# Berghojo/bmhrl

Measured on AMD Instinct MI355X. Metric: caption-train steps/sec, higher is better.
Workload: dtype bf16; 1 GPU; BMHRL warmstart step (BASELINE configs[1]): B=16/GPU Tv=256 Ta=800 L=30 V=10172 N=2 d_model=1024 H=4 dropout=0.1; global_batch=16, parallelism=dp1, launch=hip-graph

## Files before the change

### bmhrl_amd/_lib.py

```python
from __future__ import annotations

import ctypes as C
import os

_HERE = os.path.dirname(os.path.abspath(__file__))
LIB_PATH = os.environ.get("BMHRL_HIP_LIB") or os.path.join(_HERE, "csrc", "libbmhrl_hip.so")

i32, i64, u64, f32, f64 = C.c_int32, C.c_int64, C.c_uint64, C.c_float, C.c_double
ptr = C.c_void_p


class RnnLayer(C.Structure):
    _fields_ = [("w_ih", C.c_void_p), ("w_hh", C.c_void_p), ("b_ih", C.c_void_p), ("b_hh", C.c_void_p),
                ("in_seq", C.c_void_p), ("in_ld", C.c_int64), ("in_dim", C.c_int32), ("gates", C.c_int32),
                ("seq_out", C.c_void_p), ("h", C.c_void_p * 2), ("c", C.c_void_p * 2),
                ("arelu_alpha", C.c_void_p), ("arelu_beta", C.c_void_p), ("xproj", C.c_void_p)]


class FusionTailParams(C.Structure):
    _fields_ = [(n, C.c_void_p) for n in ("gamma_ca", "beta_ca", "gamma_cv", "beta_cv", "a_v",
                                          "dgamma_ca", "dbeta_ca", "dgamma_cv", "dbeta_cv", "da_v")]


class GemmDesc(C.Structure):
# ... 114 lines not shown
    "bmhrl_consensus": [ptr, i64, i32, i32, i32, i64, i32, ptr, i32, ptr, ptr, ptr],
    "bmhrl_word_cost": [ptr, i64, ptr, i64, i64, f32, i32, i32, i32, i32, ptr, ptr, ptr, ptr, ptr, ptr, ptr, ptr],
    "bmhrl_lsa_match": [ptr, i64, i64, i64, ptr, i32, i32, i32, ptr, ptr],
    "bmhrl_word_loss": [ptr, ptr, ptr, ptr, ptr, ptr, ptr, f32, i32, i32, i32, i32, ptr, ptr, ptr, ptr],
    "bmhrl_word_loss_bwd": [ptr, i64, ptr, ptr, ptr, ptr, ptr, ptr, ptr, i64, i32, i32, i32, ptr],
    "bmhrl_proposal_assign": [ptr, i32, ptr, i32, f32, i32, i32, ptr, ptr, ptr, ptr, ptr],
    "bmhrl_proposal_head": [ptr, ptr, f32, i32, i32, i32, ptr, i64, i64, ptr, ptr, ptr, ptr, f32, f32, ptr, ptr, ptr, ptr, ptr,
                            ptr],
    "bmhrl_proposal_select": [ptr, i32, i64, ptr, i32, f32, ptr, ptr, ptr, i64, ptr],
    "bmhrl_tiou_hits": [ptr, i32, ptr, i32, ptr, ptr, ptr, i32, ptr, i32, i32, ptr, i64, ptr, i64, ptr],
    "bmhrl_tiou_pairs": [ptr, i32, ptr, i32, ptr, ptr, ptr, i32, f64, ptr, i64, ptr, i64, ptr],
    "bmhrl_crop_segments": [ptr, ptr, ptr, i32, i32, i32, ptr, ptr, i32, f32, i32, ptr, ptr, ptr, ptr, ptr],
    "bmhrl_rollout_advantage": [ptr, i64, i32, i32, i32, i64, ptr, i64, i32, ptr, ptr, ptr, ptr, ptr, i64, ptr, ptr],
    "bmhrl_policy_loss_fwd": [ptr, i64, ptr, ptr, ptr, f32, ptr, ptr, ptr, i64, i32, ptr],
    "bmhrl_policy_loss_bwd": [ptr, i64, ptr, ptr, ptr, f32, ptr, ptr, ptr, ptr, i64, i64, i32, ptr],
    "bmhrl_ngram_stats": [ptr, i32, ptr, i32, ptr, i32, ptr, ptr],
}

QUERIES = {
    "bmhrl_hip_arch": (C.c_char_p, []),
    "bmhrl_hip_abi_version": (C.c_int, []),
    "bmhrl_deterministic_enabled": (C.c_int, []),
    "bmhrl_layernorm_bwd_workspace": (C.c_int64, [i64, i32]),
    "bmhrl_attention_shared128_bwd_workspace": (C.c_int64, [i32, i32, i32]),
    "bmhrl_attention_max_keys": (C.c_int, []),
    "bmhrl_attention_config": (C.c_int, [i32, i32]),
    "bmhrl_attention_plan": (C.c_int, [i32, i32, i32, i32, i32, i64]),
    "bmhrl_attention_bwd_scores256_ok": (C.c_int, [i32, i32, i32, i64]),
    "bmhrl_memory_attention_ok": (C.c_int, [i32, i32, i32]),
    "bmhrl_small_attention_ok": (C.c_int, [i32, i32, i32]),
    "bmhrl_gemm_splits": (C.c_int, [i32, i32, i32, i32]),
    "bmhrl_gemm_plan": (C.c_int, [C.POINTER(GemmDesc), C.POINTER(i32)]),
    "bmhrl_gemm_group_plan": (C.c_int, [C.POINTER(GemmDesc), i32]),
    "bmhrl_gemm_f32_fast_path": (C.c_int, [C.POINTER(GemmDesc)]),
}


def _is_pointer(t) -> bool:
    return t is ptr or isinstance(t, type(C.POINTER(i32)))


PTR_SLOTS = {name: tuple(i for i, t in enumerate(argtypes) if _is_pointer(t))
             for name, argtypes in [*PROTOTYPES.items(), *((name, q[1]) for name, q in QUERIES.items())]}

_lib = None


def load() -> C.CDLL:
    global _lib
    if _lib is not None:
        return _lib
    if not os.path.exists(LIB_PATH):
        raise RuntimeError(
            f"{LIB_PATH} is missing: build it with `python -m bmhrl_amd.build` (hipcc --offload-arch=gfx950). "
            "bmhrl_amd has no CPU fallback.")
    import torch
    hip_rt = os.path.join(os.path.dirname(torch.__file__), "lib", "libamdhip64.so")
    if os.path.exists(hip_rt):
        C.CDLL(hip_rt, mode=C.RTLD_GLOBAL)
    lib = C.CDLL(LIB_PATH)

    def bind(name, restype, argtypes):
        try:
            fn = getattr(lib, name)
        except AttributeError:
            raise RuntimeError(f"{LIB_PATH} does not export {name}: it was built from older sources than this package; "
# ... 21 lines not shown
```

### bmhrl_amd/csrc/gemm.hip

```cpp
#include <cstdlib>
#include <algorithm>
#include <type_traits>

#include "common.h"
#include "../../include/bmhrl_hip.h"

namespace {

struct GemmArgs {
  int M, N, K, batch2;
  const bf16_t* A; long lda, a_sb1, a_sb2;
  const bf16_t* B; long ldb, b_sb1, b_sb2;
  float* C; long ldc, c_sb1, c_sb2;
  bf16_t* Cb; long ldcb, cb_sb1, cb_sb2;
  int epilogue; float alpha; int relu; int accumulate;
  const float* bias;
  const float* residual; long ldr, r_sb1, r_sb2;
  const uint8_t* mask; long mask_sb1, mask_sm;
  const float* rowvec; const float* rowvec2; long rv_sb1, rv_sb2;
  const bf16_t* aux; long ldaux, aux_sb1, aux_sb2;
  float dropout_p; uint64_t seed; const uint64_t* seed_dev; long drop_sb1, drop_sb2, drop_sm;
  float* colsum; long cs_sb2, bias_sb2, cs_sb1, bias_sb1;
  int tiles_m, splits, k_per_split, vec_ok, dbg, fast_bf16, fast_pd, fast_f32, tiles_mn;
  int xcd_chunk, group_m;
// ... 606 lines not shown
  r /= p.tiles_mn;
  gemm_body<TM, TN, AT, BT>(p, bx, r % p.splits, r / p.splits);
}


template <int N> struct IC { static constexpr int value = N; };
template <int I, int N, class F>
__device__ __forceinline__ void gsfor(F&& f) {
  if constexpr (I < N) {
    f(IC<I>{});
    gsfor<I + 1, N>(f);
  }
}
template <int IMM>
__device__ __forceinline__ void gemm_glds16(const char* src, char* dst) {
  __builtin_amdgcn_global_load_lds((const __attribute__((address_space(1))) void*)src,
                                   (__attribute__((address_space(3))) void*)dst, 16, IMM, 0);
}

template <int OFF>
__device__ __forceinline__ bf16x8 gemm_lds128(unsigned addr) {
  bf16x8 r;
  asm volatile("ds_read_b128 %0, %1 offset:%2" : "=v"(r) : "v"(addr), "n"(OFF));
  return r;
}
template <int OFF>
__device__ __forceinline__ bf16x4 gemm_ldstr(unsigned addr) {
  bf16x4 r;
  asm volatile("ds_read_b64_tr_b16 %0, %1 offset:%2" : "=v"(r) : "v"(addr), "n"(OFF));
  return r;
}

template <int TM, int TN, bool AT, bool BT, int NS>
__global__ __launch_bounds__(256, 2) void gemm_glds_kernel(const GemmArgs p) {
  constexpr int BM = 64 * TM, BN = 64 * TN;
  constexpr int A_BYTES = BM * BK * 2, B_BYTES = BN * BK * 2, STAGE_BYTES = A_BYTES + B_BYTES;
  constexpr int EPI_ELEMS = BM * (BN + 4) * 2;
  constexpr int SMEM_ELEMS = (NS * STAGE_BYTES / 2) > EPI_ELEMS ? (NS * STAGE_BYTES / 2) : EPI_ELEMS;

  __shared__ __attribute__((aligned(16))) bf16_t smem[SMEM_ELEMS];
  char* const sbase = reinterpret_cast<char*>(smem);
  const unsigned lds0 = (unsigned)(uintptr_t)(__attribute__((address_space(3))) char*)sbase;

  const int tid = threadIdx.x, lane = tid & 63;
  const int wave = __builtin_amdgcn_readfirstlane(tid >> 6);
  const int wm = wave >> 1, wn = wave & 1;
  const int r32 = lane & 31, h = lane >> 5;
  const int g1 = (lane >> 4) & 1, q4 = (lane & 15) >> 2, p4 = lane & 3;
  const int bz = blockIdx.z, b1 = bz / p.batch2, b2 = bz % p.batch2;
  int tile_m, tile_n;
  tile_of_block(p, (int)blockIdx.x, tile_m, tile_n);
  const int m0 = tile_m * BM, n0 = tile_n * BN;
  const char* __restrict__ Ag = reinterpret_cast<const char*>(p.A + b1 * p.a_sb1 + b2 * p.a_sb2);
  const char* __restrict__ Bg = reinterpret_cast<const char*>(p.B + b1 * p.b_sb1 + b2 * p.b_sb2);
  const int M8 = (p.M + 7) & ~7, N8 = (p.N + 7) & ~7;
  const int k_begin = blockIdx.y * p.k_per_split;
  const int k_end = min(p.K, k_begin + p.k_per_split);
  const int nk = (k_end - k_begin) / BK;
  if (nk <= 0) return;
  BMHRL_GSTAMP(0)

  constexpr int PA = A_BYTES / 1024 / 4, PB = B_BYTES / 1024 / 4;
  unsigned a_off[PA], b_off[PB];
  auto piece_off = [&](const bool trans, const int R, const int i, const int r0, const int rmax, const int rmax8, const long ld) {
    if (!trans) {
      const int row = wave * (R / 4) + 8 * i + (lane >> 3), pc = lane & 7;
      const int sc = pc ^ ((row >> 1) & 7);
      return (unsigned)((long)min(r0 + row, rmax - 1) * ld * 2 + sc * 16);
    }
    const int cpr = R / 8, rpp = 64 / cpr;
    const int krow = wave * 16 + rpp * i + lane / cpr, pc = lane % cpr;
    const int sc = pc ^ (R == 128 ? ((krow & 3) << 2) : (((krow >> 1) & 1) << 2));
    return (unsigned)((long)krow * ld * 2 + (long)min(r0 + sc * 8, rmax8 - 8) * 2);
  };
#pragma unroll
  for (int i = 0; i < PA; ++i) a_off[i] = piece_off(AT, BM, i, m0, p.M, M8, p.lda);
#pragma unroll
  for (int i = 0; i < PB; ++i) b_off[i] = piece_off(BT, BN, i, n0, p.N, N8, p.ldb);
  const long a_step = AT ? (long)BK * p.lda * 2 : (long)BK * 2, b_step = BT ? (long)BK * p.ldb * 2 : (long)BK * 2;
  const char* const a_k0 = Ag + (AT ? (long)k_begin * p.lda * 2 : (long)k_begin * 2);
  const char* const b_k0 = Bg + (BT ? (long)k_begin * p.ldb * 2 : (long)k_begin * 2);
  char* const a_dst = sbase + wave * PA * 1024;
  char* const b_dst = sbase + A_BYTES + wave * PB * 1024;
  auto stage = [&](auto st_, const int t) {
    constexpr int ST = decltype(st_)::value;
    auto sgpr_ptr = [](const char* q) {
      const uint64_t u = reinterpret_cast<uint64_t>(q);
      const uint32_t lo = __builtin_amdgcn_readfirstlane((uint32_t)u), hi = __builtin_amdgcn_readfirstlane((uint32_t)(u >> 32));
      return reinterpret_cast<const char*>(((uint64_t)hi << 32) | lo);
    };
    const char* ab = sgpr_ptr(a_k0 + (long)t * a_step);
    const char* bb = sgpr_ptr(b_k0 + (long)t * b_step);
    gsfor<0, PA>([&](auto i) {
      constexpr int I = decltype(i)::value;
      unsigned o = a_off[I];
      asm volatile("" : "+v"(o));
      gemm_glds16<0>(ab + o, a_dst + ST * STAGE_BYTES + I * 1024);
    });
    gsfor<0, PB>([&](auto i) {
      constexpr int I = decltype(i)::value;
      unsigned o = b_off[I];
      asm volatile("" : "+v"(o));
      gemm_glds16<0>(bb + o, b_dst + ST * STAGE_BYTES + I * 1024);
    });
  };

  constexpr int NA = AT ? TM : 4, NB = BT ? TN : 4;
  unsigned a_addr0[NA], b_addr0[NB];
  if constexpr (!AT) {
#pragma unroll
    for (int ks = 0; ks < 4; ++ks) a_addr0[ks] = lds0 + (wm * 32 * TM + r32) * 128 + (((2 * ks + h) ^ ((r32 >> 1) & 7)) << 4);
  } else {
    constexpr int RB = BM * 2;
#pragma unroll
    for (int i = 0; i < TM; ++i) {
      const int c = wm * 4 * TM + 4 * i + 2 * g1 + (p4 >> 1);
      const int sw = BM == 128 ? (q4 << 2) : (((q4 >> 1) & 1) << 2);
      a_addr0[i] = lds0 + (8 * h + q4) * RB + ((c ^ sw) << 4) + ((p4 & 1) << 3);
    }
  }
  if constexpr (!BT) {
#pragma unroll
    for (int ks = 0; ks < 4; ++ks) b_addr0[ks] = lds0 + A_BYTES + (wn * 32 * TN + r32) * 128 + (((2 * ks + h) ^ ((r32 >> 1) & 7)) << 4);
  } else {
    constexpr int RB = BN * 2;
#pragma unroll
    for (int i = 0; i < TN; ++i) {
      const int c = wn * 4 * TN + 4 * i + 2 * g1 + (p4 >> 1);
      const int sw = BN == 128 ? (q4 << 2) : (((q4 >> 1) & 1) << 2);
      b_addr0[i] = lds0 + A_BYTES + (8 * h + q4) * RB + ((c ^ sw) << 4) + ((p4 & 1) << 3);
    }
  }

  f32x16 acc[TM][TN];
#pragma unroll
  for (int i = 0; i < TM; ++i)
#pragma unroll
    for (int j = 0; j < TN; ++j)
#pragma unroll
      for (int r = 0; r < 16; ++r) acc[i][j][r] = 0.f;

  constexpr int RA = AT ? 2 : 1, RBn = BT ? 2 : 1;
  constexpr int PER_KS = TM * RA + TN * RBn;
  auto compute = [&](auto st_) {
    constexpr int ST = decltype(st_)::value;
    bf16x8 af[4][TM], bfr[4][TN];
    unsigned a_addr[1][NA], b_addr[1][NB];
#pragma unroll
    for (int i = 0; i < NA; ++i) a_addr[0][i] = a_addr0[i] + ST * STAGE_BYTES;
#pragma unroll
    for (int i = 0; i < NB; ++i) b_addr[0][i] = b_addr0[i] + ST * STAGE_BYTES;
    auto read_ks = [&](auto ks_) {
      constexpr int KS = decltype(ks_)::value;
      gsfor<0, TM>([&](auto i_) {
        constexpr int I = decltype(i_)::value;
        if constexpr (!AT) {
          af[KS][I] = gemm_lds128<I * 32 * 128>(a_addr[0][KS]);
        } else {
          constexpr int RB = BM * 2;
          af[KS][I] = join8(gemm_ldstr<KS * 16 * RB>(a_addr[0][I]), gemm_ldstr<(KS * 16 + 4) * RB>(a_addr[0][I]));
        }
      });
      gsfor<0, TN>([&](auto i_) {
        constexpr int I = decltype(i_)::value;
        if constexpr (!BT) {
          bfr[KS][I] = gemm_lds128<I * 32 * 128>(b_addr[0][KS]);
        } else {
          constexpr int RB = BN * 2;
          bfr[KS][I] = join8(gemm_ldstr<KS * 16 * RB>(b_addr[0][I]), gemm_ldstr<(KS * 16 + 4) * RB>(b_addr[0][I]));
        }
      });
    };
    read_ks(IC<0>{});
    read_ks(IC<1>{});
    gsfor<0, 4>([&](auto ks_) {
      constexpr int KS = decltype(ks_)::value;
      constexpr int LEFT = KS < 3 ? PER_KS : 0;
      __builtin_amdgcn_sched_barrier(0);
      bf16x8& a0 = af[KS][0];
      bf16x8& b0 = bfr[KS][0];
      bf16x8& a1 = af[KS][TM - 1];
      bf16x8& b1r = bfr[KS][TN - 1];
      if constexpr (TM == 2 && TN == 2) asm volatile("s_waitcnt lgkmcnt(%4)" : "+v"(a0), "+v"(a1), "+v"(b0), "+v"(b1r) : "n"(LEFT));
      else asm volatile("s_waitcnt lgkmcnt(%2)" : "+v"(a0), "+v"(b0) : "n"(LEFT));
      __builtin_amdgcn_sched_barrier(0);
#pragma unroll
      for (int mi = 0; mi < TM; ++mi)
#pragma unroll
        for (int ni = 0; ni < TN; ++ni)
          acc[mi][ni] = __builtin_amdgcn_mfma_f32_32x32x16_bf16(af[KS][mi], bfr[KS][ni], acc[mi][ni], 0, 0, 0);
      if constexpr (KS + 2 < 4) read_ks(IC<KS + 2>{});
    });
  };

  constexpr int PT = PA + PB;
  auto step = [&](auto st_, const int t) {
    constexpr int ST = decltype(st_)::value;
    constexpr int NXT = (ST + NS - 1) % NS;
    const bool more = t + NS - 1 < nk;
    if (more) stage(IC<NXT>{}, t + NS - 1);
    compute(st_);
    if (t + 1 < nk) {
      if (more && NS > 2) asm volatile("s_waitcnt vmcnt(%0)" ::"n"((NS - 2) * PT) : "memory");
      else asm volatile("s_waitcnt vmcnt(0)" ::: "memory");
      __builtin_amdgcn_s_barrier();
      asm volatile("" ::: "memory");
    }
  };
  gsfor<0, NS - 1>([&](auto i_) {
    if (decltype(i_)::value < nk) stage(i_, decltype(i_)::value);
  });
  BMHRL_GSTAMP(1)
  if (NS > 2 && nk > 1) asm volatile("s_waitcnt vmcnt(%0)" ::"n"((NS - 2) * PT) : "memory");
  if (NS == 2 || nk < NS - 1) asm volatile("s_waitcnt vmcnt(0)" ::: "memory");
  __builtin_amdgcn_s_barrier();
  asm volatile("" ::: "memory");
  BMHRL_GSTAMP(2)
  for (int t0 = 0; t0 < nk; t0 += NS) {
    gsfor<0, NS>([&](auto i_) {
      if (t0 + decltype(i_)::value < nk) step(i_, t0 + decltype(i_)::value);
    });
  }
  asm volatile("s_waitcnt lgkmcnt(0)" ::: "memory");
  __builtin_amdgcn_s_barrier();
  asm volatile("" ::: "memory");
  BMHRL_GSTAMP(3)
  gemm_epilogue<TM, TN, SMEM_ELEMS>(p, acc, smem, b1, b2, m0, n0, (int)blockIdx.y);
  BMHRL_GSTAMP(4)
}

template <bool AT, bool BT>
__global__ __launch_bounds__(512, 2) void gemm_glds8_kernel(const GemmArgs p) {
  constexpr int TM = 2, TN = 2, NS = 3, NW = 8;
  constexpr int BM = 128, BN = 128;
  constexpr int A_BYTES = BM * BK * 2, B_BYTES = BN * BK * 2, STAGE_BYTES = A_BYTES + B_BYTES;
  constexpr int EPI_ELEMS = BM * (BN + 4) * 2;
  constexpr int SMEM_ELEMS = (NS * STAGE_BYTES / 2) > EPI_ELEMS ? (NS * STAGE_BYTES / 2) : EPI_ELEMS;
  static_assert(4 * 64 * 256 <= SMEM_ELEMS * 2, "the partial tile of wave group 1 fits the stages");

  __shared__ __attribute__((aligned(16))) bf16_t smem[SMEM_ELEMS];
  char* const sbase = reinterpret_cast<char*>(smem);
  const unsigned lds0 = (unsigned)(uintptr_t)(__attribute__((address_space(3))) char*)sbase;

  const int tid = threadIdx.x, lane = tid & 63;
  const int wave = __builtin_amdgcn_readfirstlane(tid >> 6);
  const int grp = wave >> 2, w4 = wave & 3;
  const int wm = w4 >> 1, wn = w4 & 1;
  const int r32 = lane & 31, h = lane >> 5;
  const int g1 = (lane >> 4) & 1, q4 = (lane & 15) >> 2, p4 = lane & 3;
  const int bz = blockIdx.z, b1 = bz / p.batch2, b2 = bz % p.batch2;
  const int tile_m = blockIdx.x % p.tiles_m, tile_n = blockIdx.x / p.tiles_m;
  const int m0 = tile_m * BM, n0 = tile_n * BN;
  const char* __restrict__ Ag = reinterpret_cast<const char*>(p.A + b1 * p.a_sb1 + b2 * p.a_sb2);
  const char* __restrict__ Bg = reinterpret_cast<const char*>(p.B + b1 * p.b_sb1 + b2 * p.b_sb2);
  const int M8 = (p.M + 7) & ~7, N8 = (p.N + 7) & ~7;
  const int nk = p.K / BK;
  BMHRL_GSTAMP(0)

  constexpr int PA = A_BYTES / 1024 / NW, PB = B_BYTES / 1024 / NW;
  unsigned a_off[PA], b_off[PB];
  auto piece_off = [&](const bool trans, const int R, const int i, const int r0, const int rmax, const int rmax8, const long ld) {
// ... 153 lines not shown
  if (grp == 1) {
#pragma unroll
    for (int mi = 0; mi < TM; ++mi)
#pragma unroll
      for (int ni = 0; ni < TN; ++ni)
#pragma unroll
        for (int g = 0; g < 4; ++g) {
          f32x4 v;
#pragma unroll
          for (int e = 0; e < 4; ++e) v[e] = acc[mi][ni][4 * g + e];
          xch[((mi * TN + ni) * 4 + g) * 64] = v;
        }
  }
  __syncthreads();
  if (grp == 1) return;
#pragma unroll
  for (int mi = 0; mi < TM; ++mi)
#pragma unroll
    for (int ni = 0; ni < TN; ++ni)
#pragma unroll
      for (int g = 0; g < 4; ++g) {
        const f32x4 v = xch[((mi * TN + ni) * 4 + g) * 64];
#pragma unroll
        for (int e = 0; e < 4; ++e) acc[mi][ni][4 * g + e] += v[e];
      }
  __syncthreads();
  gemm_epilogue<TM, TN, SMEM_ELEMS, false>(p, acc, smem, b1, b2, m0, n0, 0);
  BMHRL_GSTAMP(4)
}

bool uses_glds(const GemmArgs& a, int a_trans, int b_trans) {
  static const int no_glds = getenv("BMHRL_GEMM_NOGLDS") ? atoi(getenv("BMHRL_GEMM_NOGLDS")) : 0;
  const long a_span = (a_trans ? 64 : (long)a.M) * a.lda * 2, b_span = (b_trans ? 64 : (long)a.N) * a.ldb * 2;
  return !no_glds && a.K % BK == 0 && a_span < (1l << 31) && b_span < (1l << 31) && a.M >= 8 && a.N >= 8;
}

enum { LOOP_REG = 0, LOOP_GLDS = 1, LOOP_GLDS8 = 2 };
enum { TILE_64 = 0, TILE_128 = 1, TILE_128x64 = 2 };
enum { SPLIT_NONE = 0, SPLIT_ATOMIC = 1, SPLIT_ORDERED = 2 };
enum { EPIPATH_FAST_BF16 = 0, EPIPATH_FAST_PD = 1, EPIPATH_GENERIC = 2 };
struct GemmPlan { int loop, tile, stages, splits, split_form, epi_path, vec_ok, ordered_colsum, fast_f32; };

template <int TM, int TN>
hipError_t launch(const GemmArgs& a, const GemmPlan& pl, int a_trans, int b_trans, int batch, hipStream_t s) {
  GemmArgs p = a;
  constexpr int BM = 64 * TM, BN = 64 * TN;
  const int splits = pl.splits;
  p.tiles_m = (a.M + BM - 1) / BM;
  const int tiles_n = (a.N + BN - 1) / BN;
  p.tiles_mn = p.tiles_m * tiles_n;
  p.xcd_chunk = p.group_m = 0;
  {
    static const int xcd = getenv("BMHRL_GEMM_XCD") ? atoi(getenv("BMHRL_GEMM_XCD")) : 0;
    if (xcd && p.tiles_mn % 8 == 0 && p.tiles_mn >= 64 && tiles_n >= 2) {
      const int chunk = p.tiles_mn / 8;
      int g = 1;
      while ((g + 1) * (g + 1) <= chunk && g + 1 <= p.tiles_m) ++g;
      while (g > 1 && chunk % g != 0) --g;
      if (xcd >= 2) g = xcd <= p.tiles_m ? xcd : p.tiles_m;
      p.xcd_chunk = chunk;
      p.group_m = g;
    }
  }
  p.splits = splits;
  p.dbg = getenv("BMHRL_GEMM_DBG") ? atoi(getenv("BMHRL_GEMM_DBG")) : 0;
  const int ktiles = (a.K + BK - 1) / BK;
  p.k_per_split = ((ktiles + splits - 1) / splits) * BK;
  dim3 grid(p.tiles_m * tiles_n, splits, batch), block(256);
  if constexpr (TM == 2 && TN == 2) {
    if (pl.loop == LOOP_GLDS8) {
      dim3 block8(512);
      if (!a_trans && !b_trans) hipLaunchKernelGGL((gemm_glds8_kernel<false, false>), grid, block8, 0, s, p);
      else if (!a_trans && b_trans) hipLaunchKernelGGL((gemm_glds8_kernel<false, true>), grid, block8, 0, s, p);
      else if (a_trans && !b_trans) hipLaunchKernelGGL((gemm_glds8_kernel<true, false>), grid, block8, 0, s, p);
// ... 156 lines not shown
                                       : d->residual ? (d->dropout_p > 0.f || !d->Cb) : (d->dropout_p == 0.f && !d->Cb);
  a.fast_f32 = fast_f32_on && d->C && d->epilogue == BMHRL_EPI_LINEAR && !d->mask && !d->aux && !d->rowvec && !d->rowvec2 &&
               !d->relu && !d->colsum && f32_combo && a.vec_ok;
  const bool out_ok = d->Cb && !d->C && !d->residual && !d->colsum && !d->accumulate && !d->bias && al(d->Cb, 16) &&
                      d->ldcb % 8 == 0 && d->cb_sb1 % 8 == 0 && d->cb_sb2 % 8 == 0 && d->rowvec;
  a.fast_pd = (d->epilogue == BMHRL_EPI_PROB && out_ok && d->rowvec2 && (!d->mask || d->mask_sm == 0) && !d->aux) ||
              (d->epilogue == BMHRL_EPI_DSCORE && out_ok && d->aux && al(d->aux, 16) && d->ldaux % 8 == 0 &&
               d->aux_sb1 % 8 == 0 && d->aux_sb2 % 8 == 0 && (!d->mask || d->mask_sm == 0));
  const bool can_split = d->allow_split_k && d->C && !d->Cb && d->epilogue == BMHRL_EPI_LINEAR && !d->relu && !d->mask &&
                         d->dropout_p == 0.f && (!d->accumulate || d->split_ws) && !d->colsum;
  tp = tile_plan(d->M, d->N, d->K, batch, can_split);
  a.split_ws = (tp.splits > 1 && d->split_ws && d->split_ws_elems >= (int64_t)tp.splits * batch * d->M * d->N) ? d->split_ws : nullptr;
  if (tp.splits > 1 && d->accumulate && !a.split_ws) return -22;
  return 0;
}

int plan_problem(const bmhrl_gemm_desc* d, GemmArgs& a, GemmPlan& pl, int& batch) {
  TilePlan tp;
  if (const int rc = prepare(d, a, tp, batch)) return rc;
  const int TM = tp.mid || tp.big ? 2 : 1, TN = tp.big && !tp.mid ? 2 : 1;
  pl.tile = tp.mid ? TILE_128x64 : tp.big ? TILE_128 : TILE_64;
  pl.splits = tp.splits;
  pl.loop = LOOP_REG;
  pl.stages = 2;
  if (uses_glds(a, d->a_trans, d->b_trans)) {
    static const int force_ns = getenv("BMHRL_GEMM_STAGES") ? atoi(getenv("BMHRL_GEMM_STAGES")) : 0;
    const long blocks = (long)((d->M + 64 * TM - 1) / (64 * TM)) * ((d->N + 64 * TN - 1) / (64 * TN)) * batch;
    int ns = TM == 1 && tp.splits == 1 && blocks <= 448 ? 4 : 2;
    if (force_ns) ns = TM == 1 ? (force_ns >= 4 ? 4 : 2) : 2;
    pl.loop = LOOP_GLDS;
    pl.stages = ns;
    static const int w8 = getenv("BMHRL_GEMM_W8") ? atoi(getenv("BMHRL_GEMM_W8")) : 0;
    static const long w8_max = getenv("BMHRL_GEMM_W8MAX") ? atol(getenv("BMHRL_GEMM_W8MAX")) : 256;
    if (TM == 2 && TN == 2 && w8 && tp.splits == 1 && d->K >= 2 * BK && (w8 == 2 || blocks <= w8_max)) {
      pl.loop = LOOP_GLDS8;
      pl.stages = 3;
    }
  }
  pl.split_form = tp.splits == 1 ? SPLIT_NONE : a.split_ws ? SPLIT_ORDERED : SPLIT_ATOMIC;
  pl.epi_path = tp.splits == 1 && a.fast_bf16 ? EPIPATH_FAST_BF16 : tp.splits == 1 && a.fast_pd ? EPIPATH_FAST_PD : EPIPATH_GENERIC;
  if (tp.splits != 1 || pl.loop == LOOP_GLDS8) a.fast_f32 = 0;
  pl.fast_f32 = a.fast_f32;
  pl.vec_ok = a.vec_ok;
  pl.ordered_colsum = bmhrl_deterministic() && a.colsum != nullptr;
  return 0;
}

int group_prepare(const bmhrl_gemm_desc* d, int n, GemmGroup& g, int& total) {
  GemmArgs* ps[4] = {&g.p0, &g.p1, &g.p2, &g.p3};
  bool same = n > 1;
  total = 0;
  for (int i = 0; i < n; ++i) {
    GemmPlan pl;
    int batch;
    if (const int rc = plan_problem(d + i, *ps[i], pl, batch)) return rc;
    GemmArgs& p = *ps[i];
    same = same && pl.tile == TILE_64 && pl.loop == LOOP_REG && d[i].a_trans == d[0].a_trans && d[i].b_trans == d[0].b_trans &&
           pl.split_form != SPLIT_ORDERED && !pl.ordered_colsum;
    p.tiles_m = (p.M + 63) / 64;
    p.tiles_mn = p.tiles_m * ((p.N + 63) / 64);
    p.splits = pl.splits;
    p.dbg = 0;
    const int ktiles = (p.K + BK - 1) / BK;
    p.k_per_split = ((ktiles + pl.splits - 1) / pl.splits) * BK;
    g.first[i] = total;
    total += p.tiles_mn * pl.splits * batch;
  }
  return same ? 1 : 0;
}
}

extern "C" int bmhrl_gemm_plan(const bmhrl_gemm_desc* d, int32_t plan[8]) {
  GemmArgs a;
  GemmPlan pl;
  int batch;
  if (const int rc = plan_problem(d, a, pl, batch)) return rc;
  if (plan) {
    plan[0] = pl.loop; plan[1] = pl.tile; plan[2] = pl.stages; plan[3] = pl.splits;
    plan[4] = pl.split_form; plan[5] = pl.epi_path; plan[6] = pl.vec_ok; plan[7] = pl.ordered_colsum;
  }
  return 0;
}

extern "C" int bmhrl_gemm_f32_fast_path(const bmhrl_gemm_desc* d) {
  GemmArgs a;
  GemmPlan pl;
  int batch;
  if (const int rc = plan_problem(d, a, pl, batch)) return rc;
  return pl.fast_f32;
}

extern "C" int bmhrl_gemm_group_plan(const bmhrl_gemm_desc* d, int32_t n) {
  BMHRL_CHECK_ARG(d && n >= 1);
  int launches = 0;
  for (int i = 0; i < n; i += 4) {
    GemmGroup g;
    int total;
    const int rc = group_prepare(d + i, n - i < 4 ? n - i : 4, g, total);
    if (rc < 0) return rc;
    launches += rc;
  }
  return launches;
}

void gemm_trace_dump(const GemmArgs& a, hipStream_t stream) {
#ifdef BMHRL_GEMM_TRACE
  if (getenv("BMHRL_GEMM_TRACE")) {
    long long hh[2][8];
    (void)hipStreamSynchronize(stream);
    (void)hipMemcpyFromSymbol(hh, HIP_SYMBOL(g_gemm_trace), sizeof(hh));
    for (int w = 0; w < 2; ++w)
      fprintf(stderr, "gemm trace (%s block, M %d N %d K %d): setup %lld  first tile %lld  loop %lld  epilogue %lld  total %lld\n",
              w ? "last" : "first", a.M, a.N, a.K, hh[w][1] - hh[w][0], hh[w][2] - hh[w][1], hh[w][3] - hh[w][2], hh[w][4] - hh[w][3],
              hh[w][4] - hh[w][0]);
  }
#else
  (void)a; (void)stream;
#endif
}

extern "C" int bmhrl_gemm(const bmhrl_gemm_desc* d, bmhrl_stream_t stream) {
  GemmArgs a;
  GemmPlan pl;
  int batch;
  if (const int rc = plan_problem(d, a, pl, batch)) return rc;
  GemmArgs full = a;
  if (pl.ordered_colsum) a.colsum = nullptr;
  hipError_t e;
  if (pl.tile == TILE_128x64) e = launch<2, 1>(a, pl, d->a_trans, d->b_trans, batch, (hipStream_t)stream);
  else if (pl.tile == TILE_128) e = launch<2, 2>(a, pl, d->a_trans, d->b_trans, batch, (hipStream_t)stream);
  else e = launch<1, 1>(a, pl, d->a_trans, d->b_trans, batch, (hipStream_t)stream);
  if (e == hipSuccess && pl.ordered_colsum) {
    hipLaunchKernelGGL(colsum_ordered_kernel, dim3((unsigned)((full.N + 63) / 64)), dim3(1024), 0, (hipStream_t)stream, full, d->batch1);
    e = hipGetLastError();
  }
  if (e == hipSuccess && pl.split_form == SPLIT_ORDERED) {
    GemmArgs r = a;
    r.splits = pl.splits;
    const int ktiles = (a.K + BK - 1) / BK, tiles_per_split = (ktiles + pl.splits - 1) / pl.splits;
    const int n_live = (ktiles + tiles_per_split - 1) / tiles_per_split;
    const long total = (long)batch * a.M * a.N;
    hipLaunchKernelGGL(splitk_reduce_kernel, dim3((unsigned)std::min<long>((total + 255) / 256, 2048)), dim3(256), 0, (hipStream_t)stream, r, batch,
                       n_live);
    e = hipGetLastError();
  }
  gemm_trace_dump(a, (hipStream_t)stream);
  return hip_status(e);
}

extern "C" int bmhrl_gemm_group(const bmhrl_gemm_desc* d, int32_t n, bmhrl_stream_t stream) {
  BMHRL_CHECK_ARG(d && n >= 1);
  if (n > 4) {
    for (int i = 0; i < n; i += 4)
      if (const int rc = bmhrl_gemm_group(d + i, n - i < 4 ? n - i : 4, stream)) return rc;
    return 0;
  }
  GemmGroup g;
  int total;
  const int same = group_prepare(d, n, g, total);
  if (same < 0) return same;
  if (!same) {
    for (int i = 0; i < n; ++i)
      if (const int rc = bmhrl_gemm(d + i, stream)) return rc;
    return 0;
  }
  GemmArgs* ps[4] = {&g.p0, &g.p1, &g.p2, &g.p3};
  for (int i = n; i < 5; ++i) g.first[i] = total;
  for (int i = n; i < 4; ++i) *ps[i] = g.p0;
  g.n = n;
  dim3 grid((unsigned)total), block(256);
  const hipStream_t s = (hipStream_t)stream;
  if (!d[0].a_trans && !d[0].b_trans) hipLaunchKernelGGL((gemm_group_kernel<1, 1, false, false>), grid, block, 0, s, g);
  else if (!d[0].a_trans && d[0].b_trans) hipLaunchKernelGGL((gemm_group_kernel<1, 1, false, true>), grid, block, 0, s, g);
  else if (d[0].a_trans && !d[0].b_trans) hipLaunchKernelGGL((gemm_group_kernel<1, 1, true, false>), grid, block, 0, s, g);
  else hipLaunchKernelGGL((gemm_group_kernel<1, 1, true, true>), grid, block, 0, s, g);
  return hip_status(hipGetLastError());
}
```

### bmhrl_amd/ops.py

```python
from __future__ import annotations

import ctypes as C
import math
import os
from typing import Optional, Tuple

import numpy as np
import torch

from . import _lib

EPI_LINEAR, EPI_PROB, EPI_DSCORE, EPI_RELU_BWD = 0, 1, 2, 3


def pad8(n: int) -> int:
    return (n + 7) & ~7


def stream() -> int:
    return torch._C._cuda_getCurrentRawStream(torch.cuda.current_device())


_Tensor, _Parameter = torch.Tensor, torch.nn.Parameter
_TENSORS = frozenset((_Tensor, _Parameter))
# ... 91 lines not shown
    d.bias_sb2 = bias_sb2; d.bias_sb1 = bias_sb1; d.colsum_sb1 = colsum_sb1
    d.split_ws = _ptr(split_ws); d.split_ws_elems = 0 if split_ws is None else split_ws.numel()
    return d


_GEMM_OPERANDS = ("C_f32", "C_bf16", "bias", "residual", "mask", "rowvec", "rowvec2", "aux", "seed_dev", "colsum")


def gemm(A: torch.Tensor, B: torch.Tensor, M: int, N: int, K: int, *, defer: Optional[list] = None, **desc) -> None:
    d = gemm_desc(A, B, M, N, K, **desc)
    if defer is not None and _GROUP_LEAVES:
        defer.append((d, (A, B, *map(desc.get, _GEMM_OPERANDS))))
        return
    _launch("bmhrl_gemm", C.byref(d))


GEMM_PLAN_FIELDS = ("loop", "tile", "stages", "splits", "split_form", "epi_path", "vec_ok", "ordered_colsum")


def gemm_plan(d: "_lib.GemmDesc") -> dict:
    plan = (_lib.i32 * 8)()
    _lib.check(_query("bmhrl_gemm_plan", C.byref(d), plan), "bmhrl_gemm_plan")
    return dict(zip(GEMM_PLAN_FIELDS, plan))


def gemm_f32_fast_path(d: "_lib.GemmDesc") -> bool:
    return bool(_query("bmhrl_gemm_f32_fast_path", C.byref(d)))


def gemm_group_plan(descs) -> int:
    return int(_query("bmhrl_gemm_group_plan", (_lib.GemmDesc * len(descs))(*descs), len(descs)))


_GROUP_LEAVES = os.environ.get("BMHRL_GEMM_GROUP", "1") == "1"


def gemm_flush(deferred: list) -> None:
    if not deferred:
        return
    _launch("bmhrl_gemm_group", (_lib.GemmDesc * len(deferred))(*[d for d, _ in deferred]), len(deferred))
    deferred.clear()


_SPLITS = {}


def gemm_splits(M: int, N: int, K: int, batch: int = 1) -> int:
    key = (M, N, K, batch)
    r = _SPLITS.get(key)
    if r is None:
        r = int(_query("bmhrl_gemm_splits", M, N, K, batch, refusal=False))
        if r < 1:
            raise RuntimeError(f"bmhrl_gemm_splits{key} failed: {r}")
        _SPLITS[key] = r
    return r


def gemm_overwrites(M: int, N: int, K: int, batch: int = 1) -> bool:
    return gemm_splits(M, N, K, batch) == 1


def attention_fwd(Q, K, V, O, row_max, row_sum, mask, mask_sb, mask_sq, B, H, Sq, Sk, dk, scale, ldq, ldk, ldv, ldo,
                  q_off=0, k_off=0, v_off=0, dropout_p=0.0, seed=0, seed_dev=None):
    f16 = Q.dtype == torch.float16
    if any((t.dtype == torch.float16) != f16 for t in (K, V, O)):
        raise RuntimeError("attention_fwd: Q, K, V and O must share one 16-bit type")
# ... 1040 lines not shown
```

### include/bmhrl_hip.h

```cpp
#ifndef BMHRL_HIP_H
#define BMHRL_HIP_H

#include <stdint.h>

#ifdef __cplusplus
extern "C" {
#endif

typedef void* bmhrl_stream_t;

enum {
  BMHRL_EPI_LINEAR = 0,
  BMHRL_EPI_PROB = 1,
  BMHRL_EPI_DSCORE = 2,
  BMHRL_EPI_RELU_BWD = 3
};

typedef struct bmhrl_gemm_desc {
  int32_t M, N, K;
  int32_t batch1, batch2;
  const void* A; int64_t lda, a_sb1, a_sb2; int32_t a_trans;
  const void* B; int64_t ldb, b_sb1, b_sb2; int32_t b_trans;
  float* C;  int64_t ldc, c_sb1, c_sb2;
  void* Cb;  int64_t ldcb, cb_sb1, cb_sb2;
  int32_t epilogue;
  float alpha;
  int32_t relu;
  int32_t accumulate;
  int32_t allow_split_k;
  const float* bias;
  const float* residual; int64_t ldr, r_sb1, r_sb2;
  const uint8_t* mask; int64_t mask_sb1, mask_sm;
  const float* rowvec; const float* rowvec2; int64_t rv_sb1, rv_sb2;
  const void* aux; int64_t ldaux, aux_sb1, aux_sb2;
  float dropout_p; uint64_t seed;
  int64_t drop_sb1, drop_sb2, drop_sm;
  const uint64_t* seed_dev;
  float* colsum; int64_t colsum_sb2;
  int64_t bias_sb2;
  int64_t colsum_sb1, bias_sb1;
  float* split_ws; int64_t split_ws_elems;
} bmhrl_gemm_desc;

int bmhrl_gemm(const bmhrl_gemm_desc* d, bmhrl_stream_t stream);
int bmhrl_gemm_group(const bmhrl_gemm_desc* descs, int32_t n, bmhrl_stream_t stream);
int bmhrl_gemm_splits(int32_t M, int32_t N, int32_t K, int32_t batch);
int bmhrl_gemm_plan(const bmhrl_gemm_desc* d, int32_t plan[8]);
int bmhrl_gemm_f32_fast_path(const bmhrl_gemm_desc* d);
int bmhrl_gemm_group_plan(const bmhrl_gemm_desc* descs, int32_t n);

int bmhrl_attention_fwd(const void* Q, int64_t ldq, const void* K, int64_t ldk, const void* V, int64_t ldv,
                        void* O, int64_t ldo, float* row_max, float* row_sum, const uint8_t* mask, int64_t mask_sb,
                        int64_t mask_sq,
                        int32_t B, int32_t H, int32_t Sq, int32_t Sk, int32_t DK, float scale,
                        float dropout_p, uint64_t seed, const uint64_t* seed_dev, bmhrl_stream_t stream);

int bmhrl_attention_shared128_fwd(const void* Qp, int64_t ldq, const void* X, int64_t ldx, void* ctx, int64_t ldo,
                                  float* row_max, float* row_sum, const uint8_t* mask, int64_t mask_sb,
                                  int32_t B, int32_t H, int32_t Sq, int32_t Sk, float scale, bmhrl_stream_t stream);

int bmhrl_attention_fwd_f16(const void* Q, int64_t ldq, const void* K, int64_t ldk, const void* V, int64_t ldv,
                            void* O, int64_t ldo, float* row_max, float* row_sum, const uint8_t* mask, int64_t mask_sb,
                            int64_t mask_sq, int32_t B, int32_t H, int32_t Sq, int32_t Sk, int32_t DK, float scale,
                            float dropout_p, uint64_t seed, const uint64_t* seed_dev, bmhrl_stream_t stream);
int bmhrl_attention_shared128_fwd_f16(const void* Qp, int64_t ldq, const void* X, int64_t ldx, void* ctx, int64_t ldo,
                                      float* row_max, float* row_sum, const uint8_t* mask, int64_t mask_sb,
                                      int32_t B, int32_t H, int32_t Sq, int32_t Sk, float scale, bmhrl_stream_t stream);

int64_t bmhrl_attention_shared128_bwd_workspace(int32_t B, int32_t H, int32_t Sk);
int bmhrl_attention_shared128_bwd(const void* Qp, int64_t ldq, const void* X, int64_t ldx, const void* dCx, int64_t lddo,
                                  const float* row_max, const float* row_sum, const float* delta, const uint8_t* mask,
                                  int64_t mask_sb, void* dQp, int64_t lddq, float* dX, int64_t lddx, int32_t accumulate_dx,
                                  float* workspace, int32_t B, int32_t H, int32_t Sq, int32_t Sk, float scale,
                                  bmhrl_stream_t stream);

int bmhrl_attention_max_keys(void);

int bmhrl_attention_config(int32_t head_dim, int32_t code);

int bmhrl_attention_plan(int32_t kind, int32_t B, int32_t H, int32_t Sq, int32_t Sk, int64_t mask_sq);

int bmhrl_small_attention_ok(int32_t Sq, int32_t Sk, int32_t dk);
// ... 360 lines not shown
```

Before: 212.8 steps/s (one step = one B=16 batch on one GPU; whole-job aggregate over all GPUs).

## Route grouped GEMMs through LDS-direct pipeline and support ragged K tails

Moves the GEMM main loop into a reusable device body and adds a grouped kernel variant that uses the global-to-LDS pipelined loop instead of the register loop for grouped launches. The same path now accepts K that is a multiple of 16 but not of the block K, by clamping loads on the last ragged tile and running fewer k-substeps there. When a group already has enough tiles, split-K is dropped and the stage count is picked from the total block count. The aim is to give grouped and ragged-K GEMMs the faster pipelined loop and to avoid split-K reduction overhead. The cost is extra template instantiations, plus the risk of wrong results or lower occupancy from the ragged-tail clamping.

```diff
diff --git a/bmhrl_amd/_lib.py b/bmhrl_amd/_lib.py
--- a/bmhrl_amd/_lib.py
+++ b/bmhrl_amd/_lib.py
@@ -170,6 +170,7 @@
     "bmhrl_gemm_splits": (C.c_int, [i32, i32, i32, i32]),
     "bmhrl_gemm_plan": (C.c_int, [C.POINTER(GemmDesc), C.POINTER(i32)]),
     "bmhrl_gemm_group_plan": (C.c_int, [C.POINTER(GemmDesc), i32]),
+    "bmhrl_gemm_group_member_plan": (C.c_int, [C.POINTER(GemmDesc), i32, i32, C.POINTER(i32)]),
     "bmhrl_gemm_f32_fast_path": (C.c_int, [C.POINTER(GemmDesc)]),
 }
 
diff --git a/bmhrl_amd/csrc/gemm.hip b/bmhrl_amd/csrc/gemm.hip
--- a/bmhrl_amd/csrc/gemm.hip
+++ b/bmhrl_amd/csrc/gemm.hip
@@ -662,7 +662,7 @@
 }
 
 template <int TM, int TN, bool AT, bool BT, int NS>
-__global__ __launch_bounds__(256, 2) void gemm_glds_kernel(const GemmArgs p) {
+__device__ __forceinline__ void gemm_glds_body(const GemmArgs& p, const int bx, const int by, const int bz) {
   constexpr int BM = 64 * TM, BN = 64 * TN;
   constexpr int A_BYTES = BM * BK * 2, B_BYTES = BN * BK * 2, STAGE_BYTES = A_BYTES + B_BYTES;
   constexpr int EPI_ELEMS = BM * (BN + 4) * 2;
@@ -677,42 +677,45 @@
   const int wm = wave >> 1, wn = wave & 1;
   const int r32 = lane & 31, h = lane >> 5;
   const int g1 = (lane >> 4) & 1, q4 = (lane & 15) >> 2, p4 = lane & 3;
-  const int bz = blockIdx.z, b1 = bz / p.batch2, b2 = bz % p.batch2;
+  const int b1 = bz / p.batch2, b2 = bz % p.batch2;
   int tile_m, tile_n;
-  tile_of_block(p, (int)blockIdx.x, tile_m, tile_n);
+  tile_of_block(p, bx, tile_m, tile_n);
   const int m0 = tile_m * BM, n0 = tile_n * BN;
   const char* __restrict__ Ag = reinterpret_cast<const char*>(p.A + b1 * p.a_sb1 + b2 * p.a_sb2);
   const char* __restrict__ Bg = reinterpret_cast<const char*>(p.B + b1 * p.b_sb1 + b2 * p.b_sb2);
   const int M8 = (p.M + 7) & ~7, N8 = (p.N + 7) & ~7;
-  const int k_begin = blockIdx.y * p.k_per_split;
+  const int k_begin = by * p.k_per_split;
   const int k_end = min(p.K, k_begin + p.k_per_split);
-  const int nk = (k_end - k_begin) / BK;
+  const int nk = (k_end - k_begin + BK - 1) / BK;
+  const int r_live = ((k_end - k_begin) & (BK - 1)) >> 4;
+  const int t_rag = r_live ? nk - 1 : -1;
   if (nk <= 0) return;
   BMHRL_GSTAMP(0)
 
   constexpr int PA = A_BYTES / 1024 / 4, PB = B_BYTES / 1024 / 4;
   unsigned a_off[PA], b_off[PB];
-  auto piece_off = [&](const bool trans, const int R, const int i, const int r0, const int rmax, const int rmax8, const long ld) {
+  auto piece_off = [&](const bool trans, const int R, const int i, const int r0, const int rmax, const int rmax8, const long ld,
+                       const int klive) {
     if (!trans) {
       const int row = wave * (R / 4) + 8 * i + (lane >> 3), pc = lane & 7;
-      const int sc = pc ^ ((row >> 1) & 7);
+      const int sc = min(pc ^ ((row >> 1) & 7), (klive >> 3) - 1);
       return (unsigned)((long)min(r0 + row, rmax - 1) * ld * 2 + sc * 16);
     }
     const int cpr = R / 8, rpp = 64 / cpr;
     const int krow = wave * 16 + rpp * i + lane / cpr, pc = lane % cpr;
     const int sc = pc ^ (R == 128 ? ((krow & 3) << 2) : (((krow >> 1) & 1) << 2));
-    return (unsigned)((long)krow * ld * 2 + (long)min(r0 + sc * 8, rmax8 - 8) * 2);
-  };
-#pragma unroll
-  for (int i = 0; i < PA; ++i) a_off[i] = piece_off(AT, BM, i, m0, p.M, M8, p.lda);
-#pragma unroll
-  for (int i = 0; i < PB; ++i) b_off[i] = piece_off(BT, BN, i, n0, p.N, N8, p.ldb);
+    return (unsigned)((long)min(krow, klive - 1) * ld * 2 + (long)min(r0 + sc * 8, rmax8 - 8) * 2);
+  };
+#pragma unroll
+  for (int i = 0; i < PA; ++i) a_off[i] = piece_off(AT, BM, i, m0, p.M, M8, p.lda, BK);
+#pragma unroll
+  for (int i = 0; i < PB; ++i) b_off[i] = piece_off(BT, BN, i, n0, p.N, N8, p.ldb, BK);
   const long a_step = AT ? (long)BK * p.lda * 2 : (long)BK * 2, b_step = BT ? (long)BK * p.ldb * 2 : (long)BK * 2;
   const char* const a_k0 = Ag + (AT ? (long)k_begin * p.lda * 2 : (long)k_begin * 2);
   const char* const b_k0 = Bg + (BT ? (long)k_begin * p.ldb * 2 : (long)k_begin * 2);
   char* const a_dst = sbase + wave * PA * 1024;
   char* const b_dst = sbase + A_BYTES + wave * PB * 1024;
-  auto stage = [&](auto st_, const int t) {
+  auto issue = [&](auto st_, const int t, const unsigned (&ao)[PA], const unsigned (&bo)[PB]) {
     constexpr int ST = decltype(st_)::value;
     auto sgpr_ptr = [](const char* q) {
       const uint64_t u = reinterpret_cast<uint64_t>(q);
@@ -723,16 +726,28 @@
     const char* bb = sgpr_ptr(b_k0 + (long)t * b_step);
     gsfor<0, PA>([&](auto i) {
       constexpr int I = decltype(i)::value;
-      unsigned o = a_off[I];
+      unsigned o = ao[I];
       asm volatile("" : "+v"(o));
       gemm_glds16<0>(ab + o, a_dst + ST * STAGE_BYTES + I * 1024);
     });
     gsfor<0, PB>([&](auto i) {
       constexpr int I = decltype(i)::value;
-      unsigned o = b_off[I];
+      unsigned o = bo[I];
       asm volatile("" : "+v"(o));
       gemm_glds16<0>(bb + o, b_dst + ST * STAGE_BYTES + I * 1024);
     });
+  };
+  auto stage = [&](auto st_, const int t) {
+    if (t == t_rag) {
+      unsigned al[PA], bl[PB];
+#pragma unroll
+      for (int i = 0; i < PA; ++i) al[i] = piece_off(AT, BM, i, m0, p.M, M8, p.lda, 16 * r_live);
+#pragma unroll
+      for (int i = 0; i < PB; ++i) bl[i] = piece_off(BT, BN, i, n0, p.N, N8, p.ldb, 16 * r_live);
+      issue(st_, t, al, bl);
+    } else {
+      issue(st_, t, a_off, b_off);
+    }
   };
 
   constexpr int NA = AT ? TM : 4, NB = BT ? TN : 4;
@@ -772,8 +787,8 @@
 
   constexpr int RA = AT ? 2 : 1, RBn = BT ? 2 : 1;
   constexpr int PER_KS = TM * RA + TN * RBn;
-  auto compute = [&](auto st_) {
-    constexpr int ST = decltype(st_)::value;
+  auto compute = [&](auto st_, auto nks_) {
+    constexpr int ST = decltype(st_)::value, NKS = decltype(nks_)::value;
     bf16x8 af[4][TM], bfr[4][TN];
     unsigned a_addr[1][NA], b_addr[1][NB];
 #pragma unroll
@@ -802,10 +817,10 @@
       });
     };
     read_ks(IC<0>{});
-    read_ks(IC<1>{});
-    gsfor<0, 4>([&](auto ks_) {
+    if constexpr (NKS > 1) read_ks(IC<1>{});
+    gsfor<0, NKS>([&](auto ks_) {
       constexpr int KS = decltype(ks_)::value;
-      constexpr int LEFT = KS < 3 ? PER_KS : 0;
+      constexpr int LEFT = KS + 1 < NKS ? PER_KS : 0;
       __builtin_amdgcn_sched_barrier(0);
       bf16x8& a0 = af[KS][0];
       bf16x8& b0 = bfr[KS][0];
@@ -819,7 +834,7 @@
 #pragma unroll
         for (int ni = 0; ni < TN; ++ni)
           acc[mi][ni] = __builtin_amdgcn_mfma_f32_32x32x16_bf16(af[KS][mi], bfr[KS][ni], acc[mi][ni], 0, 0, 0);
-      if constexpr (KS + 2 < 4) read_ks(IC<KS + 2>{});
+      if constexpr (KS + 2 < NKS) read_ks(IC<KS + 2>{});
     });
   };
 
@@ -829,7 +844,13 @@
     constexpr int NXT = (ST + NS - 1) % NS;
     const bool more = t + NS - 1 < nk;
     if (more) stage(IC<NXT>{}, t + NS - 1);
-    compute(st_);
+    if (t == t_rag) {
+      if (r_live == 1) compute(st_, IC<1>{});
+      else if (r_live == 2) compute(st_, IC<2>{});
+      else compute(st_, IC<3>{});
+    } else {
+      compute(st_, IC<4>{});
+    }
     if (t + 1 < nk) {
       if (more && NS > 2) asm volatile("s_waitcnt vmcnt(%0)" ::"n"((NS - 2) * PT) : "memory");
       else asm volatile("s_waitcnt vmcnt(0)" ::: "memory");
@@ -855,8 +876,30 @@
   __builtin_amdgcn_s_barrier();
   asm volatile("" ::: "memory");
   BMHRL_GSTAMP(3)
-  gemm_epilogue<TM, TN, SMEM_ELEMS>(p, acc, smem, b1, b2, m0, n0, (int)blockIdx.y);
+  gemm_epilogue<TM, TN, SMEM_ELEMS>(p, acc, smem, b1, b2, m0, n0, by);
   BMHRL_GSTAMP(4)
+}
+
+template <int TM, int TN, bool AT, bool BT, int NS>
+__global__ __launch_bounds__(256, 2) void gemm_glds_kernel(const GemmArgs p) {
+  gemm_glds_body<TM, TN, AT, BT, NS>(p, (int)blockIdx.x, (int)blockIdx.y, (int)blockIdx.z);
+}
+
+template <bool AT, bool BT, int NS>
+__global__ __launch_bounds__(256, 2) void gemm_glds_group_kernel(const GemmGroup g) {
+  const int b = (int)blockIdx.x;
+  int i = 0;
+  if (g.n > 1 && b >= g.first[1]) i = 1;
+  if (g.n > 2 && b >= g.first[2]) i = 2;
+  if (g.n > 3 && b >= g.first[3]) i = 3;
+  GemmArgs p = g.p0;
+  if (i == 1) p = g.p1;
+  if (i == 2) p = g.p2;
+  if (i == 3) p = g.p3;
+  int r = b - g.first[i];
+  const int bx = r % p.tiles_mn;
+  r /= p.tiles_mn;
+  gemm_glds_body<1, 1, AT, BT, NS>(p, bx, r % p.splits, r / p.splits);
 }
 
 template <bool AT, bool BT>
@@ -1076,14 +1119,18 @@
 bool uses_glds(const GemmArgs& a, int a_trans, int b_trans) {
   static const int no_glds = getenv("BMHRL_GEMM_NOGLDS") ? atoi(getenv("BMHRL_GEMM_NOGLDS")) : 0;
   const long a_span = (a_trans ? 64 : (long)a.M) * a.lda * 2, b_span = (b_trans ? 64 : (long)a.N) * a.ldb * 2;
-  return !no_glds && a.K % BK == 0 && a_span < (1l << 31) && b_span < (1l << 31) && a.M >= 8 && a.N >= 8;
+  const bool k_ok = a.K % BK == 0 || (a.K % 16 == 0 && a.K >= 192);
+  return !no_glds && k_ok && a_span < (1l << 31) && b_span < (1l << 31) && a.M >= 8 && a.N >= 8;
 }
 
 enum { LOOP_REG = 0, LOOP_GLDS = 1, LOOP_GLDS8 = 2 };
 enum { TILE_64 = 0, TILE_128 = 1, TILE_128x64 = 2 };
 enum { SPLIT_NONE = 0, SPLIT_ATOMIC = 1, SPLIT_ORDERED = 2 };
 enum { EPIPATH_FAST_BF16 = 0, EPIPATH_FAST_PD = 1, EPIPATH_GENERIC = 2 };
-struct GemmPlan { int loop, tile, stages, splits, split_form, epi_path, vec_ok, ordered_colsum, fast_f32; };
+struct GemmPlan {
+  int loop, tile, stages, splits, split_form, epi_path, vec_ok, ordered_colsum, fast_f32;
+  int fast_f32_unsplit;
+};
 
 template <int TM, int TN>
 hipError_t launch(const GemmArgs& a, const GemmPlan& pl, int a_trans, int b_trans, int batch, hipStream_t s) {
@@ -1306,13 +1353,14 @@
     pl.stages = ns;
     static const int w8 = getenv("BMHRL_GEMM_W8") ? atoi(getenv("BMHRL_GEMM_W8")) : 0;
     static const long w8_max = getenv("BMHRL_GEMM_W8MAX") ? atol(getenv("BMHRL_GEMM_W8MAX")) : 256;
-    if (TM == 2 && TN == 2 && w8 && tp.splits == 1 && d->K >= 2 * BK && (w8 == 2 || blocks <= w8_max)) {
+    if (TM == 2 && TN == 2 && w8 && tp.splits == 1 && d->K >= 2 * BK && d->K % BK == 0 && (w8 == 2 || blocks <= w8_max)) {
       pl.loop = LOOP_GLDS8;
       pl.stages = 3;
     }
   }
   pl.split_form = tp.splits == 1 ? SPLIT_NONE : a.split_ws ? SPLIT_ORDERED : SPLIT_ATOMIC;
   pl.epi_path = tp.splits == 1 && a.fast_bf16 ? EPIPATH_FAST_BF16 : tp.splits == 1 && a.fast_pd ? EPIPATH_FAST_PD : EPIPATH_GENERIC;
+  pl.fast_f32_unsplit = pl.loop == LOOP_GLDS8 ? 0 : a.fast_f32;
   if (tp.splits != 1 || pl.loop == LOOP_GLDS8) a.fast_f32 = 0;
   pl.fast_f32 = a.fast_f32;
   pl.vec_ok = a.vec_ok;
@@ -1320,25 +1368,48 @@
   return 0;
 }
 
-int group_prepare(const bmhrl_gemm_desc* d, int n, GemmGroup& g, int& total) {
+int group_prepare(const bmhrl_gemm_desc* d, int n, GemmGroup& g, int& total, GemmPlan (&pls)[4]) {
   GemmArgs* ps[4] = {&g.p0, &g.p1, &g.p2, &g.p3};
+  int batch[4];
   bool same = n > 1;
+  long tiles = 0;
+  for (int i = 0; i < n; ++i) {
+    if (const int rc = plan_problem(d + i, *ps[i], pls[i], batch[i])) return rc;
+    GemmArgs& p = *ps[i];
+    const GemmPlan& pl = pls[i];
+    same = same && pl.tile == TILE_64 && (pl.loop == LOOP_REG || pl.loop == LOOP_GLDS) && pl.loop == pls[0].loop &&
+           d[i].a_trans == d[0].a_trans && d[i].b_trans == d[0].b_trans && !pl.ordered_colsum;
+    p.tiles_m = (p.M + 63) / 64;
+    p.tiles_mn = p.tiles_m * ((p.N + 63) / 64);
+    p.xcd_chunk = p.group_m = 0;
+    p.dbg = 0;
+    tiles += (long)p.tiles_mn * batch[i];
+  }
+  const bool drop = same && tiles >= 192;
+  bool split = false;
   total = 0;
   for (int i = 0; i < n; ++i) {
-    GemmPlan pl;
-    int batch;
-    if (const int rc = plan_problem(d + i, *ps[i], pl, batch)) return rc;
     GemmArgs& p = *ps[i];
-    same = same && pl.tile == TILE_64 && pl.loop == LOOP_REG && d[i].a_trans == d[0].a_trans && d[i].b_trans == d[0].b_trans &&
-           pl.split_form != SPLIT_ORDERED && !pl.ordered_colsum;
-    p.tiles_m = (p.M + 63) / 64;
-    p.tiles_mn = p.tiles_m * ((p.N + 63) / 64);
+    GemmPlan& pl = pls[i];
+    if (drop && pl.splits > 1) {
+      pl.splits = 1;
+      pl.split_form = SPLIT_NONE;
+      pl.fast_f32 = p.fast_f32 = pl.fast_f32_unsplit;
+      p.split_ws = nullptr;
+    }
+    same = same && pl.split_form != SPLIT_ORDERED;
+    split = split || pl.splits > 1;
     p.splits = pl.splits;
-    p.dbg = 0;
     const int ktiles = (p.K + BK - 1) / BK;
     p.k_per_split = ((ktiles + pl.splits - 1) / pl.splits) * BK;
     g.first[i] = total;
-    total += p.tiles_mn * pl.splits * batch;
+    total += p.tiles_mn * pl.splits * batch[i];
+  }
+  if (same && pls[0].loop == LOOP_GLDS) {
+    static const int force_ns = getenv("BMHRL_GEMM_STAGES") ? atoi(getenv("BMHRL_GEMM_STAGES")) : 0;
+    int ns = !split && total <= 448 ? 4 : 2;
+    if (force_ns) ns = force_ns >= 4 ? 4 : 2;
+    for (int i = 0; i < n; ++i) pls[i].stages = ns;
   }
   return same ? 1 : 0;
 }
@@ -1369,12 +1440,30 @@
   int launches = 0;
   for (int i = 0; i < n; i += 4) {
     GemmGroup g;
+    GemmPlan pls[4];
     int total;
-    const int rc = group_prepare(d + i, n - i < 4 ? n - i : 4, g, total);
+    const int rc = group_prepare(d + i, n - i < 4 ? n - i : 4, g, total, pls);
     if (rc < 0) return rc;
     launches += rc;
   }
   return launches;
+}
+
+extern "C" int bmhrl_gemm_group_member_plan(const bmhrl_gemm_desc* d, int32_t n, int32_t member, int32_t plan[8]) {
+  BMHRL_CHECK_ARG(d && n >= 1 && member >= 0 && member < n);
+  const int first = member / 4 * 4;
+  GemmGroup g;
+  GemmPlan pls[4];
+  int total;
+  const int rc = group_prepare(d + first, n - first < 4 ? n - first : 4, g, total, pls);
+  if (rc < 0) return rc;
+  if (rc == 0) return bmhrl_gemm_plan(d + member, plan);
+  const GemmPlan& pl = pls[member - first];
+  if (plan) {
+    plan[0] = pl.loop; plan[1] = pl.tile; plan[2] = pl.stages; plan[3] = pl.splits;
+    plan[4] = pl.split_form; plan[5] = pl.epi_path; plan[6] = pl.vec_ok; plan[7] = pl.ordered_colsum;
+  }
+  return 0;
 }
 
 void gemm_trace_dump(const GemmArgs& a, hipStream_t stream) {
@@ -1430,8 +1519,9 @@
     return 0;
   }
   GemmGroup g;
+  GemmPlan pls[4];
   int total;
-  const int same = group_prepare(d, n, g, total);
+  const int same = group_prepare(d, n, g, total, pls);
   if (same < 0) return same;
   if (!same) {
     for (int i = 0; i < n; ++i)
@@ -1444,6 +1534,19 @@
   g.n = n;
   dim3 grid((unsigned)total), block(256);
   const hipStream_t s = (hipStream_t)stream;
+  if (pls[0].loop == LOOP_GLDS) {
+#define BMHRL_GLDS_GROUP(AT_, BT_)                                                                            \
+    do {                                                                                                        \
+      if (pls[0].stages == 4) hipLaunchKernelGGL((gemm_glds_group_kernel<AT_, BT_, 4>), grid, block, 0, s, g); \
+      else hipLaunchKernelGGL((gemm_glds_group_kernel<AT_, BT_, 2>), grid, block, 0, s, g);                    \
+    } while (0)
+    if (!d[0].a_trans && !d[0].b_trans) BMHRL_GLDS_GROUP(false, false);
+    else if (!d[0].a_trans && d[0].b_trans) BMHRL_GLDS_GROUP(false, true);
+    else if (d[0].a_trans && !d[0].b_trans) BMHRL_GLDS_GROUP(true, false);
+    else BMHRL_GLDS_GROUP(true, true);
+#undef BMHRL_GLDS_GROUP
+    return hip_status(hipGetLastError());
+  }
   if (!d[0].a_trans && !d[0].b_trans) hipLaunchKernelGGL((gemm_group_kernel<1, 1, false, false>), grid, block, 0, s, g);
   else if (!d[0].a_trans && d[0].b_trans) hipLaunchKernelGGL((gemm_group_kernel<1, 1, false, true>), grid, block, 0, s, g);
   else if (d[0].a_trans && !d[0].b_trans) hipLaunchKernelGGL((gemm_group_kernel<1, 1, true, false>), grid, block, 0, s, g);
diff --git a/bmhrl_amd/ops.py b/bmhrl_amd/ops.py
--- a/bmhrl_amd/ops.py
+++ b/bmhrl_amd/ops.py
@@ -147,6 +147,13 @@
     return int(_query("bmhrl_gemm_group_plan", (_lib.GemmDesc * len(descs))(*descs), len(descs)))
 
 
+def gemm_group_member_plan(descs, member: int) -> dict:
+    plan = (_lib.i32 * 8)()
+    _lib.check(_query("bmhrl_gemm_group_member_plan", (_lib.GemmDesc * len(descs))(*descs), len(descs), member, plan),
+               "bmhrl_gemm_group_member_plan")
+    return dict(zip(GEMM_PLAN_FIELDS, plan))
+
+
 _GROUP_LEAVES = os.environ.get("BMHRL_GEMM_GROUP", "1") == "1"
 
 
diff --git a/include/bmhrl_hip.h b/include/bmhrl_hip.h
--- a/include/bmhrl_hip.h
+++ b/include/bmhrl_hip.h
@@ -48,6 +48,7 @@
 int bmhrl_gemm_plan(const bmhrl_gemm_desc* d, int32_t plan[8]);
 int bmhrl_gemm_f32_fast_path(const bmhrl_gemm_desc* d);
 int bmhrl_gemm_group_plan(const bmhrl_gemm_desc* descs, int32_t n);
+int bmhrl_gemm_group_member_plan(const bmhrl_gemm_desc* descs, int32_t n, int32_t member, int32_t plan[8]);
 
 int bmhrl_attention_fwd(const void* Q, int64_t ldq, const void* K, int64_t ldk, const void* V, int64_t ldv,
                         void* O, int64_t ldo, float* row_max, float* row_sum, const uint8_t* mask, int64_t mask_sb,
```

Result: no change. 212.8 steps/s (one step = one B=16 batch on one GPU; whole-job aggregate over all GPUs) (-0.0%).
